# DeepLearnPhysics/dynamic-gcnn

Hardware: AMD Instinct MI355X
Metric: point-clouds/sec fwd+bwd at (B,N,k,C)=(24,2048,20,3), 1/2/4/8 MI355X (higher is better)
Workload: dtype f32

## Files before the change

dynamic-gcnn_amd/csrc/knn.hip:

```cpp
#include "knn_common.h"
#include <type_traits>
#include <stdlib.h>

namespace {

constexpr int ROWS = 64;
constexpr int WAVES = 4;
constexpr int TJ = 128;
constexpr int PERW = TJ / WAVES;

struct DenseClouds {
  int N;
  __host__ __device__ constexpr DenseClouds(int n) : N(n) {}
  static constexpr bool kPacked = false;
  __device__ int64_t base(int b) const { return (int64_t)b * N; }
  __device__ int size(int) const { return N; }
};
struct PackedClouds {
  const int* __restrict__ off;
  int nseg;
  static constexpr bool kPacked = true;
  __device__ int64_t base(int b) const { return off[b]; }
  __device__ int size(int b) const { return off[b + 1] - off[b]; }
  __device__ int cloud_of(int64_t row) const {
// ... 667 lines not shown
    }
  }

  __syncthreads();
  float* md = reinterpret_cast<float*>(smem_raw);
  int* mj = reinterpret_cast<int*>(smem_raw) + ROWS * KC;
#pragma unroll 1
  for (int src = 1; src < 4; ++src) {
    if (src > 1) __syncthreads();
    if (lid == src) {
#pragma unroll
      for (int t = 0; t < KC; ++t) {
        md[t * ROWS + rslot] = dl[t];
        mj[t * ROWS + rslot] = jl[t];
      }
    }
    __syncthreads();
    if (cs == 0) {
#pragma unroll 1
      for (int t = 0; t < KC; ++t) {
        const float d = (h == 0) ? md[t * ROWS + rslot] : INFINITY;
        const int j = (h == 0) ? mj[t * ROWS + rslot] : 0x7fffffff;
        const lmask_t need = key_less<true>(d, j, dl[KC - 1], jl[KC - 1]);
        if (need == 0) break;
        list_insert<KC, true>(dl, jl, d, j);
      }
    }
  }
  if (lid == 0 && row < N) {
    int32_t* out = idx + ((int64_t)b * N + row) * k;
#pragma unroll
    for (int t = 0; t < KC; ++t)
      if (t < k) out[t] = jl[t];
  }
}

__device__ __forceinline__ unsigned long long knn_key(float d, int j) {
  const unsigned u = __float_as_uint(d + 0.0f);
  const unsigned o = (u & 0x80000000u) ? ~u : (u | 0x80000000u);
  return ((unsigned long long)o << 32) | (unsigned)j;
}
__device__ __forceinline__ float knn_key_dist(unsigned long long key) {
  const unsigned o = (unsigned)(key >> 32);
  return __uint_as_float((o & 0x80000000u) ? (o & 0x7fffffffu) : ~o);
}
__device__ __forceinline__ unsigned long long readlane64(unsigned long long v, int l) {
  const unsigned lo = __builtin_amdgcn_readlane((int)(unsigned)v, l), hi = __builtin_amdgcn_readlane((int)(unsigned)(v >> 32), l);
  return ((unsigned long long)hi << 32) | lo;
}

constexpr int KA_MAXE = 8;
constexpr int KA_SLACK = 192;
constexpr int KA_SLACK_LX = 64;
constexpr float KA_C1 = 0.5f * (1.0f - 1.0f / 8192.0f);
constexpr int KA_LEVELS = 7;
__device__ __forceinline__ constexpr float ka_level(int m) {
  constexpr float L[KA_LEVELS] = {1.0f, 0.9f, 0.81f, 0.729f, 0.6561f, 0.59049f, 0.531441f};
  return L[m];
}

template <int M>
__device__ __forceinline__ unsigned xchg32(unsigned v) {
  if constexpr (M == 1) return (unsigned)__builtin_amdgcn_update_dpp((int)v, (int)v, 0xB1, 0xF, 0xF, false);
  else if constexpr (M == 2) return (unsigned)__builtin_amdgcn_update_dpp((int)v, (int)v, 0x4E, 0xF, 0xF, false);
  else if constexpr (M == 4) {
    const int t = __builtin_amdgcn_update_dpp((int)v, (int)v, 0x104, 0xF, 0x5, false);
    return (unsigned)__builtin_amdgcn_update_dpp(t, (int)v, 0x114, 0xF, 0xA, false);
  } else if constexpr (M == 8) {
    const int t = __builtin_amdgcn_update_dpp((int)v, (int)v, 0x108, 0xF, 0x3, false);
    return (unsigned)__builtin_amdgcn_update_dpp(t, (int)v, 0x118, 0xF, 0xC, false);
  } else if constexpr (M == 16) return (unsigned)__builtin_amdgcn_ds_swizzle((int)v, 0x401F);
  else return __shfl_xor(v, M, 64);
}
template <int M>
__device__ __forceinline__ unsigned long long xchg64(unsigned long long v) {
  const unsigned lo = xchg32<M>((unsigned)v), hi = xchg32<M>((unsigned)(v >> 32));
  return ((unsigned long long)hi << 32) | lo;
}
template <int J2>
__device__ __forceinline__ unsigned long long bitonic_step(unsigned long long key, int lane, bool up) {
  const unsigned long long pk = xchg64<J2>(key);
  const bool take_min = ((lane & J2) == 0) == up;
  return (take_min == (pk < key)) ? pk : key;
}
template <int J2>
__device__ __forceinline__ unsigned long long bitonic_steps_down(unsigned long long key, int lane, bool up) {
  key = bitonic_step<J2>(key, lane, up);
  if constexpr (J2 > 1) key = bitonic_steps_down<J2 / 2>(key, lane, up);
  return key;
}
__device__ __forceinline__ unsigned long long wave_merge64(unsigned long long key, int lane) {
  return bitonic_steps_down<32>(key, lane, true);
}
__device__ __forceinline__ unsigned long long wave_sort64(unsigned long long key, int lane) {
  key = bitonic_steps_down<1>(key, lane, (lane & 2) == 0);
  key = bitonic_steps_down<2>(key, lane, (lane & 4) == 0);
  key = bitonic_steps_down<4>(key, lane, (lane & 8) == 0);
  key = bitonic_steps_down<8>(key, lane, (lane & 16) == 0);
  key = bitonic_steps_down<16>(key, lane, (lane & 32) == 0);
  return wave_merge64(key, lane);
}
template <int E>
__device__ __forceinline__ unsigned long long wave_lowest64(const unsigned long long (&key)[E], int S, int lane) {
  unsigned long long res = wave_sort64(key[0], lane);
#pragma unroll
  for (int q = 1; q < E; ++q) {
// ... 241 lines not shown
      for (int s = 0; s < 4; ++s) {
        const bf16x8 a1 = *reinterpret_cast<const bf16x8*>(base + 2 * s * CS);
        acc = __builtin_amdgcn_mfma_f32_32x32x16_bf16(a1, q1[s], acc, 0, 0, 0);
        if (NPR == 3) {
          const bf16x8 a2 = *reinterpret_cast<const bf16x8*>(base + PB + 2 * s * CS);
          acc = __builtin_amdgcn_mfma_f32_32x32x16_bf16(a1, q2[s], acc, 0, 0, 0);
          acc = __builtin_amdgcn_mfma_f32_32x32x16_bf16(a2, q1[s], acc, 0, 0, 0);
        }
      }
      const float thr = (row < N) ? thr_s[rslot] : -INFINITY;
      const float gi = si * C1 - 0.5f * thr;
      const float* sj = sjs + cbase + 4 * h;
      unsigned mask = 0u;
#pragma unroll
      for (int q = 0; q < 4; ++q) {
        const float4 s4 = *reinterpret_cast<const float4*>(sj + 8 * q);
        const float sv[4] = {s4.x, s4.y, s4.z, s4.w};
#pragma unroll
        for (int e = 0; e < 4; ++e) {
          const int r = 4 * q + e;
          mask |= sel_01(m_flt(sv[e] + gi, acc[r])) << r;
        }
      }
      while (true) {
        const bool has = mask != 0u;
        const unsigned long long bal = __ballot(has);
        if (bal == 0ull) break;
        const int g = __builtin_ctz(mask | 0x80000000u) & 15;
        const int before = __builtin_amdgcn_mbcnt_hi((unsigned)(bal >> 32), __builtin_amdgcn_mbcnt_lo((unsigned)bal, 0u));
        if (has) {
          const unsigned ci = (unsigned)(cbase + (g & 3) + 8 * (g >> 2) + 4 * h);
          myq[qn + before] = LX ? (qent_t)(((unsigned)l31 << 6) | ci) : (qent_t)(((unsigned)l31 << 27) | ((unsigned)j0 + ci));
          mask &= mask - 1u;
        }
        qn += __popcll(bal);
        if (qn >= 64) {
          process(64, j0, par);
          qn -= 64;
          const qent_t mv = myq[64 + lane];
          if (lane < qn) myq[lane] = mv;
        }
      }
      if (LX && qn > 0) {
        process(qn, j0, par);
        qn = 0;
      }
    }
  }
  if (qn > 0) process(qn, 0, (nt - 1) & 1);
  __syncthreads();
  if (tid < ROWS && row0 + tid < N) cnt[grow0 + tid] = cnt_s[tid];
}

__global__ __launch_bounds__(256) void knn_select_kernel(const unsigned long long* __restrict__ ent, const int* __restrict__ cnt,
                                                         int64_t rows, int cap, int k, int32_t* __restrict__ idx) {
  const int lane = threadIdx.x & 63;
  const int64_t row = (int64_t)blockIdx.x * 4 + (threadIdx.x >> 6);
  if (row >= rows) return;
  const int S = cnt[row];
  const unsigned long long* buf = ent + row * cap;
  int32_t* out = idx + row * k;
  if (S <= 64) {
    unsigned long long key = (lane < S) ? buf[lane] : ~0ull;
    key = wave_sort64(key, lane);
    if (lane < k) out[lane] = (int32_t)(unsigned)key;
    return;
  }
  unsigned long long key[KA_MAXE];
#pragma unroll
  for (int q = 0; q < KA_MAXE; ++q) {
    const int e = lane + 64 * q;
    key[q] = (e < S) ? buf[e] : ~0ull;
  }
  const unsigned long long best = wave_lowest64<KA_MAXE>(key, S, lane);
  if (lane < k) out[lane] = (int32_t)(unsigned)best;
}

int g_knn_bf16f = -1;
int knn_bf16f_mode() {
  if (g_knn_bf16f < 0) {
    const char* e = getenv("DGCNN_KNN_BF16F");
    g_knn_bf16f = e ? ((e[0] == 'a') ? 2 : atoi(e)) : 2;
  }
  return g_knn_bf16f;
}

int g_knn_valu = 0;
bool knn_force_valu() { return g_knn_valu == 1; }

template <int LP, int MAXSTEPS, class Clouds = DenseClouds>
__global__ __launch_bounds__(256) void knn_seed_bound_kernel(const float* __restrict__ x, const float* __restrict__ sq, Clouds cl,
                                                             int64_t ldx, const int32_t* __restrict__ seed, int64_t ldseed, int k,
                                                             int64_t rows, float* __restrict__ tau0) {
  constexpr int PPS = 64 / LP;
  constexpr int RW = 2;
  const int lane = threadIdx.x & 63;
  const int64_t per = ((rows + 7) / 8 + 4 * RW - 1) / (4 * RW) * (4 * RW);
  const int64_t g0 = (int64_t)(blockIdx.x & 7) * per + ((int64_t)(blockIdx.x >> 3) * 4 + (threadIdx.x >> 6)) * RW;
  if (g0 >= rows || ((int64_t)(blockIdx.x >> 3) * 4 + (threadIdx.x >> 6)) * RW >= per) return;
  const int slot = lane / LP, cq = lane % LP;
  const int steps = (k + PPS - 1) / PPS;
  int jj[RW], nn[RW];
  int64_t gr[RW];
  const float* xc[RW];
  const float* sc[RW];
#pragma unroll
// ... 167 lines not shown
}

extern "C" int64_t dgcnn_knn_workspace_bytes(int B, int N, int C, int k) {
  if (B <= 0 || N <= 0) return 0;
  size_t n = 2 * knn_sq_bytes(B, N);
  if (dg::knn_grid_applicable(C, k)) n += dg::knn_grid_workspace_bytes(B, N);
  else if (knn_append_shape(C, k)) n += knn_append_bytes(B, N, k);
  return (int64_t)n;
}

static int g_knn_seed_min_n = -2;
static int knn_seed_min_n() {
  if (g_knn_seed_min_n == -2) {
    const char* e = getenv("DGCNN_KNN_SEED_MIN_N");
    g_knn_seed_min_n = e ? atoi(e) : -1;
  }
  return g_knn_seed_min_n;
}
extern "C" int dgcnn_knn_seed_min_n(int n) {
  const int prev = knn_seed_min_n();
  if (n >= -1) g_knn_seed_min_n = n;
  return prev;
}

static int g_knn_append = -1;
static bool knn_append_on() {
  if (g_knn_append < 0) {
    const char* e = getenv("DGCNN_KNN_APPEND");
    g_knn_append = e ? atoi(e) : 1;
  }
  return g_knn_append != 0;
}
extern "C" int dgcnn_knn_append(int on) {
  const int prev = knn_append_on() ? 1 : 0;
  if (on >= 0) g_knn_append = on ? 1 : 0;
  return prev;
}

static int g_knn_npr[2] = {-1, -1};
static int knn_append_products(bool lx) {
  if (g_knn_npr[0] < 0) {
    int a = 1, b = 1;
    const char* e = getenv("DGCNN_KNN_APPEND_NPR");
    if (e) sscanf(e, "%d,%d", &a, &b);
    g_knn_npr[0] = (a == 3) ? 3 : 1;
    g_knn_npr[1] = (b == 3) ? 3 : 1;
  }
  return g_knn_npr[lx ? 0 : 1];
}
extern "C" int dgcnn_knn_append_products(int n) {
  const int prev = knn_append_products(true);
  if (n == 1 || n == 3) g_knn_npr[0] = g_knn_npr[1] = n;
  return prev;
}

static int g_knn_hist = -1;
static int knn_hist_stride(int N) {
  if (g_knn_hist < 0) {
    const char* e = getenv("DGCNN_KNN_HIST");
    g_knn_hist = e ? atoi(e) : 2;
    if (g_knn_hist != 0 && g_knn_hist != 1 && g_knn_hist != 2 && g_knn_hist != 4) g_knn_hist = 2;
  }
  return N >= 256 ? g_knn_hist : 0;
}
extern "C" int dgcnn_knn_hist(int stride) {
  const int prev = knn_hist_stride(1 << 20);
  if (stride == 0 || stride == 1 || stride == 2 || stride == 4) g_knn_hist = stride;
  return prev;
}

static int knn_impl(const char* what, const float* x, int B, int N, int C, int64_t ldx, int k, const int32_t* seed, int64_t ldseed,
                    int kseed, int32_t* idx, void* ws, size_t ws_bytes, void* stream) {
  DG_REQUIRE(x && idx && ws, DGCNN_EINVAL, "%s: null pointer", what);
  DG_REQUIRE(B > 0 && N > 0 && C > 0 && ldx >= C, DGCNN_EINVAL, "%s: bad shape B=%d N=%d C=%d", what, B, N, C);
  DG_REQUIRE(k > 0 && k <= N, DGCNN_EINVAL, "%s: k=%d must be in [1, N=%d] (tf.nn.top_k raises otherwise)", what, k, N);
  DG_REQUIRE(k <= 64, DGCNN_EUNSUP, "%s: k=%d > 64 unsupported", what, k);
  DG_REQUIRE(C <= 128, DGCNN_EUNSUP, "%s: C=%d > 128 unsupported", what, C);
  DG_REQUIRE((reinterpret_cast<uintptr_t>(ws) & 15) == 0 && ws_bytes >= knn_sq_bytes(B, N), DGCNN_EINVAL,
             "%s: workspace must be 16-byte aligned and hold dgcnn_knn_workspace_bytes(B, N, C, k) bytes (got %zu)", what, ws_bytes);
  hipStream_t st = (hipStream_t)stream;
  float* sq_ws = reinterpret_cast<float*>(ws);
  const int64_t rows = (int64_t)B * N;
  const int vec_ok = (ldx % 4 == 0) && ((reinterpret_cast<uintptr_t>(x) & 15) == 0);
  const size_t grid_off = 2 * knn_sq_bytes(B, N);
  const bool append = knn_append_on() && knn_append_shape(C, k) && vec_ok && !knn_force_valu() && knn_bf16f_mode() != 0 &&
                      ws_bytes >= grid_off + knn_append_bytes(B, N, k);
  const int min_n = knn_seed_min_n() >= 0 ? knn_seed_min_n() : (append ? 0 : 4096);
  const bool seeded = seed && kseed >= k && kseed <= 64 && C > 4 && C <= 64 && C % 4 == 0 && vec_ok && !knn_force_valu() &&
                      N >= min_n && (int64_t)N * ldx < ((int64_t)1 << 31) && ws_bytes >= 2 * knn_sq_bytes(B, N);
  const bool grid_ws = dg::knn_grid_applicable(C, k) && !knn_force_valu() && ws_bytes >= grid_off + dg::knn_grid_workspace_bytes(B, N);
  dg::launch(sqnorm_kernel, dim3((unsigned)dg::cdiv(rows, SQ_ROWS)), dim3(256), sizeof(float) * SQ_ROWS * (C + 1), st, x,
                     ldx, rows, C, sq_ws);
  if (grid_ws && N >= dg::knn_grid_min_n())
    return dg::launch_knn_grid(x, sq_ws, B, N, C, ldx, k, idx, reinterpret_cast<char*>(ws) + grid_off, st);
  float* tau0 = nullptr;
  if (seeded) {
    tau0 = reinterpret_cast<float*>(reinterpret_cast<char*>(ws) + knn_sq_bytes(B, N));
    if (!launch_seed_bound(x, sq_ws, rows, DenseClouds(N), C, ldx, seed, ldseed, k, tau0, st)) tau0 = nullptr;
  }
  if (tau0 && append) {
    char* base = reinterpret_cast<char*>(ws) + grid_off;
    int* cnt = reinterpret_cast<int*>(base);
    unsigned long long* ent = reinterpret_cast<unsigned long long*>(base + (((size_t)rows * sizeof(int) + 255) & ~(size_t)255));
    const int cap = knn_append_cap(k, N);
    const dim3 grid((unsigned)dg::cdiv(N, ROWS), (unsigned)B);
    const int npr = knn_append_products(knn_append_lx(N));
    const int tmask = knn_append_tighten_mask(knn_append_lx(N));
#define DG_KA(LXV, NPRV) dg::launch((knn_bf16a_kernel<LXV, NPRV>), grid, dim3(256), 0, st, x, (const float*)sq_ws, N, C, ldx, k, (const float*)tau0, cap, ent, cnt, tmask)
    if (knn_append_lx(N)) { if (npr == 1) DG_KA(true, 1); else DG_KA(true, 3); }
    else { if (npr == 1) DG_KA(false, 1); else DG_KA(false, 3); }
#undef DG_KA
    dg::launch(knn_select_kernel, dim3((unsigned)dg::cdiv(rows, 4)), dim3(256), 0, st, (const unsigned long long*)ent, (const int*)cnt, rows,
               cap, k, idx);
    return dg::check_launch(what);
  }
  if (C <= 4) {
    const int hs = knn_hist_stride(N);
    if (hs > 0 && !knn_force_valu() && k <= 64 && N >= 4 * k * hs && ws_bytes >= 2 * knn_sq_bytes(B, N)) {
      float* tb = reinterpret_cast<float*>(reinterpret_cast<char*>(ws) + knn_sq_bytes(B, N));
      const dim3 hg((unsigned)dg::cdiv(N, 64), (unsigned)B);
      if (hs == 1) dg::launch(knn_hist_bound_kernel<1>, hg, dim3(256), 0, st, x, (const float*)sq_ws, N, C, ldx, k, tb);
      else if (hs == 2) dg::launch(knn_hist_bound_kernel<2>, hg, dim3(256), 0, st, x, (const float*)sq_ws, N, C, ldx, k, tb);
      else dg::launch(knn_hist_bound_kernel<4>, hg, dim3(256), 0, st, x, (const float*)sq_ws, N, C, ldx, k, tb);
      tau0 = tb;
    }
    return dispatch_k<4>(x, sq_ws, B, N, C, ldx, k, vec_ok, idx, tau0, st);
  }
  if (C <= 16) return dispatch_k<16>(x, sq_ws, B, N, C, ldx, k, vec_ok, idx, tau0, st);
  if (C <= 64) return dispatch_k<64>(x, sq_ws, B, N, C, ldx, k, vec_ok, idx, tau0, st);
  return dispatch_k<128>(x, sq_ws, B, N, C, ldx, k, vec_ok, idx, tau0, st);
}

extern "C" int dgcnn_knn_f32(const float* x, int B, int N, int C, int64_t ldx, int k, int32_t* idx,
                             void* ws, size_t ws_bytes, void* stream) {
  return knn_impl("dgcnn_knn_f32", x, B, N, C, ldx, k, nullptr, 0, 0, idx, ws, ws_bytes, stream);
}

extern "C" int dgcnn_knn_seeded_f32(const float* x, int B, int N, int C, int64_t ldx, int k, const int32_t* seed, int64_t ldseed,
                                    int kseed, int32_t* idx, void* ws, size_t ws_bytes, void* stream) {
  DG_REQUIRE(!seed || (ldseed >= kseed && kseed > 0), DGCNN_EINVAL, "dgcnn_knn_seeded_f32: bad seed shape");
  return knn_impl("dgcnn_knn_seeded_f32", x, B, N, C, ldx, k, seed, ldseed, kseed, idx, ws, ws_bytes, stream);
}

extern "C" int64_t dgcnn_knn_seg_workspace_bytes(int rows, int max_n, int C, int k) {
  if (rows <= 0 || max_n <= 0) return 0;
  size_t n = 2 * knn_sq_bytes(1, rows);
  if (knn_append_shape(C, k)) n += knn_append_rows_bytes((size_t)rows, knn_append_cap(k, max_n));
  return (int64_t)n;
}

extern "C" int dgcnn_knn_seg_f32(const float* x, int64_t ldx, int C, int k, int nseg, const int32_t* seg_off, int rows, int min_n,
                                 int max_n, const int32_t* seed, int64_t ldseed, int kseed, int32_t* idx, void* ws, size_t ws_bytes,
                                 void* stream) {
  const char* what = "dgcnn_knn_seg_f32";
  DG_REQUIRE(x && idx && ws && seg_off, DGCNN_EINVAL, "%s: null pointer", what);
  DG_REQUIRE(nseg > 0 && nseg <= 65535 && rows > 0 && C > 0 && ldx >= C, DGCNN_EINVAL, "%s: bad shape nseg=%d rows=%d C=%d", what,
             nseg, rows, C);
  DG_REQUIRE(min_n > 0 && min_n <= max_n && max_n <= rows && (int64_t)min_n * nseg <= rows && (int64_t)max_n * nseg >= rows,
             DGCNN_EINVAL, "%s: cloud sizes min_n=%d max_n=%d do not fit %d rows in %d clouds", what, min_n, max_n, rows, nseg);
  DG_REQUIRE(k > 0 && k <= min_n, DGCNN_EINVAL, "%s: k=%d must be in [1, smallest cloud=%d] (tf.nn.top_k raises otherwise)", what, k,
             min_n);
  DG_REQUIRE(k <= 64, DGCNN_EUNSUP, "%s: k=%d > 64 unsupported", what, k);
  DG_REQUIRE(C <= 128, DGCNN_EUNSUP, "%s: C=%d > 128 unsupported", what, C);
  DG_REQUIRE(!seed || (ldseed >= kseed && kseed > 0), DGCNN_EINVAL, "%s: bad seed shape", what);
  DG_REQUIRE((reinterpret_cast<uintptr_t>(ws) & 15) == 0 && ws_bytes >= knn_sq_bytes(1, rows), DGCNN_EINVAL,
             "%s: workspace must be 16-byte aligned and hold dgcnn_knn_seg_workspace_bytes(rows, max_n, C, k) bytes (got %zu)", what,
             ws_bytes);
  hipStream_t st = (hipStream_t)stream;
  float* sq_ws = reinterpret_cast<float*>(ws);
  float* tb = reinterpret_cast<float*>(reinterpret_cast<char*>(ws) + knn_sq_bytes(1, rows));
  const bool tb_ok = ws_bytes >= 2 * knn_sq_bytes(1, rows);
  const PackedClouds cl{seg_off, nseg};
  const int vec_ok = (ldx % 4 == 0) && ((reinterpret_cast<uintptr_t>(x) & 15) == 0);
  const size_t aux = 2 * knn_sq_bytes(1, rows);
  const bool lx = knn_append_lx(max_n);
  const int cap = knn_append_cap(k, max_n);
  const bool append = knn_append_on() && knn_append_shape(C, k) && vec_ok && !knn_force_valu() && knn_bf16f_mode() != 0 &&
                      ws_bytes >= aux + knn_append_rows_bytes((size_t)rows, cap);
  const int seed_min = knn_seed_min_n() >= 0 ? knn_seed_min_n() : 0;
  const bool seeded = append && seed && kseed >= k && kseed <= 64 && min_n >= seed_min && (int64_t)max_n * ldx < ((int64_t)1 << 31);
  dg::launch(sqnorm_kernel, dim3((unsigned)dg::cdiv(rows, SQ_ROWS)), dim3(256), sizeof(float) * SQ_ROWS * (C + 1), st, x, ldx,
             (int64_t)rows, C, sq_ws);
  if (seeded && launch_seed_bound(x, sq_ws, (int64_t)rows, cl, C, ldx, seed, ldseed, k, tb, st)) {
    char* base = reinterpret_cast<char*>(ws) + aux;
    int* cnt = reinterpret_cast<int*>(base);
    unsigned long long* ent = reinterpret_cast<unsigned long long*>(base + (((size_t)rows * sizeof(int) + 255) & ~(size_t)255));
    const dim3 grid((unsigned)dg::cdiv(max_n, ROWS), (unsigned)nseg);
    const int npr = knn_append_products(lx);
    const int tmask = knn_append_tighten_mask(lx);
#define DG_KA(LXV, NPRV) dg::launch((knn_bf16a_kernel<LXV, NPRV, PackedClouds>), grid, dim3(256), 0, st, x, (const float*)sq_ws, cl, C, ldx, k, (const float*)tb, cap, ent, cnt, tmask)
    if (lx) { if (npr == 1) DG_KA(true, 1); else DG_KA(true, 3); }
    else { if (npr == 1) DG_KA(false, 1); else DG_KA(false, 3); }
#undef DG_KA
    dg::launch(knn_select_kernel, dim3((unsigned)dg::cdiv(rows, 4)), dim3(256), 0, st, (const unsigned long long*)ent, (const int*)cnt,
               (int64_t)rows, cap, k, idx);
    return dg::check_launch(what);
  }
  if (C <= 4) {
    const int hs = knn_hist_stride(min_n);
    const float* tau0 = nullptr;
    if (hs > 0 && !knn_force_valu() && min_n >= 4 * k * hs && tb_ok) {
      const dim3 hg((unsigned)dg::cdiv(max_n, 64), (unsigned)nseg);
      if (hs == 1) dg::launch(knn_hist_bound_kernel<1, PackedClouds>, hg, dim3(256), 0, st, x, (const float*)sq_ws, cl, C, ldx, k, tb);
      else if (hs == 2) dg::launch(knn_hist_bound_kernel<2, PackedClouds>, hg, dim3(256), 0, st, x, (const float*)sq_ws, cl, C, ldx, k, tb);
      else dg::launch(knn_hist_bound_kernel<4, PackedClouds>, hg, dim3(256), 0, st, x, (const float*)sq_ws, cl, C, ldx, k, tb);
      tau0 = tb;
    }
    return dispatch_k_packed<4>(x, sq_ws, cl, max_n, C, ldx, k, vec_ok, idx, tau0, st);
  }
  if (C <= 16) return dispatch_k_packed<16>(x, sq_ws, cl, max_n, C, ldx, k, vec_ok, idx, nullptr, st);
  if (C <= 64) return dispatch_k_packed<64>(x, sq_ws, cl, max_n, C, ldx, k, vec_ok, idx, nullptr, st);
  return dispatch_k_packed<128>(x, sq_ws, cl, max_n, C, ldx, k, vec_ok, idx, nullptr, st);
}
```

dynamic-gcnn_amd/dgcnn/_hip.py:

```python
from __future__ import annotations

import ctypes
import os

import torch

_HERE = os.path.dirname(os.path.abspath(__file__))
LIB_PATH = os.environ.get("DGCNN_HIP_LIB") or os.path.join(_HERE, "libdgcnn_hip.so")
STAT_SLOTS = 32

c_int, c_i64, c_f32, c_f64, c_vp, c_sz, c_u64 = (ctypes.c_int, ctypes.c_int64, ctypes.c_float, ctypes.c_double,
                                                  ctypes.c_void_p, ctypes.c_size_t, ctypes.c_uint64)

PROTOTYPES = {
    "dgcnn_version": [],
    "dgcnn_last_error": [],
    "dgcnn_knn_workspace_bytes": [c_int, c_int, c_int, c_int],
    "dgcnn_knn_grid": [c_int],
    "dgcnn_knn_force_valu": [c_int],
    "dgcnn_knn_bf16_filter": [c_int],
    "dgcnn_knn_f32": [c_vp, c_int, c_int, c_int, c_i64, c_int, c_vp, c_vp, c_sz, c_vp],
    "dgcnn_knn_seed_min_n": [c_int],
    "dgcnn_knn_append": [c_int],
    "dgcnn_knn_append_products": [c_int],
    "dgcnn_knn_hist": [c_int],
    "dgcnn_knn_seeded_f32": [c_vp, c_int, c_int, c_int, c_i64, c_int, c_vp, c_i64, c_int, c_vp, c_vp, c_sz, c_vp],
    "dgcnn_knn_seg_workspace_bytes": [c_int, c_int, c_int, c_int],
    "dgcnn_knn_seg_f32": [c_vp, c_i64, c_int, c_int, c_int, c_vp, c_int, c_int, c_int, c_vp, c_i64, c_int, c_vp, c_vp, c_sz, c_vp],
    "dgcnn_edge_gather_f32": [c_vp, c_i64, c_vp, c_int, c_int, c_int, c_int, c_vp, c_vp],
    "dgcnn_edge_gather_bwd_f32": [c_vp, c_vp, c_int, c_int, c_int, c_int, c_vp, c_i64, c_vp],
    "dgcnn_edge_mlp_f32": [c_vp, c_i64, c_vp, c_vp, c_int, c_int, c_int, c_int, c_int, c_vp, c_vp, c_vp],
    "dgcnn_edge_mlp_wgrad_f32": [c_vp, c_i64, c_vp, c_vp, c_int, c_int, c_int, c_int, c_int, c_vp, c_f32,
                                 c_vp, c_sz, c_vp],
    "dgcnn_edge_mlp_dgrad_scatter_f32": [c_vp, c_vp, c_vp, c_int, c_int, c_int, c_int, c_int, c_vp, c_i64, c_vp],
    "dgcnn_edge_nbr_gemm_f32": [c_vp, c_i64, c_vp, c_vp, c_vp, c_i64, c_int, c_int, c_int, c_int, c_int, c_vp, c_vp, c_vp],
    "dgcnn_edge_nbr_wgrad_f32": [c_vp, c_i64, c_vp, c_vp, c_int, c_int, c_int, c_int, c_int, c_vp, c_f32,
                                 c_vp, c_sz, c_vp],
    "dgcnn_edge_csr_build": [c_vp, c_int, c_int, c_int, c_vp, c_vp, c_vp, c_vp],
    "dgcnn_edge_gather_sum_f32": [c_vp, c_vp, c_vp, c_i64, c_int, c_vp, c_i64, c_vp],
    "dgcnn_edge_weight_split_f32": [c_vp, c_int, c_int, c_vp, c_vp],
    "dgcnn_edge_gather_add_f32": [c_vp, c_i64, c_vp, c_i64, c_vp, c_int, c_int, c_int, c_int, c_vp, c_vp, c_vp],
    "dgcnn_edge_wgrad_combine_f32": [c_vp, c_int, c_int, c_vp, c_vp],
    "dgcnn_edge_bn_act_kreduce_f32": [c_vp, c_i64, c_vp, c_i64, c_vp, c_int, c_int, c_int, c_int, c_vp, c_vp, c_vp,
                                      c_int, c_vp, c_i64, c_vp, c_i64, c_vp, c_vp],
    "dgcnn_edge_bn_bwd_reduce_f32": [c_vp, c_i64, c_vp, c_i64, c_vp, c_int, c_int, c_int, c_int, c_vp, c_vp, c_vp,
                                     c_int, c_vp, c_i64, c_vp, c_i64, c_vp, c_i64, c_vp, c_vp, c_vp],
    "dgcnn_edge_bn_bwd_reduce_points_f32": [c_vp, c_i64, c_vp, c_i64, c_vp, c_vp, c_i64, c_vp, c_i64, c_vp, c_i64, c_int,
                                            c_int, c_vp, c_vp],
    "dgcnn_edge_bn_bwd_apply_f32": [c_vp, c_i64, c_vp, c_i64, c_vp, c_int, c_int, c_int, c_int, c_vp, c_vp, c_vp,
                                    c_int, c_vp, c_i64, c_vp, c_i64, c_vp, c_i64, c_vp, c_vp, c_vp, c_vp, c_i64, c_vp,
                                    c_f32, c_vp],
    "dgcnn_edge_bn_bwd_apply_wgrad_f32": [c_vp, c_i64, c_vp, c_i64, c_vp, c_int, c_int, c_int, c_int, c_vp, c_vp, c_vp,
                                          c_vp, c_i64, c_vp, c_i64, c_vp, c_i64, c_vp, c_vp, c_vp, c_i64, c_int, c_vp, c_vp, c_f32,
                                          c_vp, c_sz, c_vp],
    "dgcnn_bn1_act_dropout_f32": [c_vp, c_i64, c_int, c_vp, c_vp, c_vp, c_int, c_f32, c_vp, c_vp, c_i64, c_vp],
    "dgcnn_bn1_bwd_dropout_f32": [c_vp, c_i64, c_int, c_vp, c_vp, c_vp, c_int, c_f32, c_vp, c_vp, c_i64, c_vp, c_vp, c_vp, c_f32, c_vp],
    "dgcnn_set_stat_slots": [c_int],
    "dgcnn_get_stat_slots": [],
    "dgcnn_gemm_set_arith": [c_int],
    "dgcnn_gemm_get_arith": [],
    "dgcnn_gemm_stat_writers": [c_int, c_int, c_int, c_int, c_vp, c_i64, c_vp, c_i64],
    "dgcnn_gemm_x3_tile_rows": [c_int, c_int, c_int],
    "dgcnn_gemm_x3_tile_cols": [c_int, c_int, c_int],
    "dgcnn_gemm_x3_tile_override": [c_int],
    "dgcnn_gemm_f32": [c_int, c_int, c_int, c_int, c_int, c_vp, c_i64, c_vp, c_i64, c_vp, c_i64, c_f32,
                       c_vp, c_i64, c_int, c_vp, c_vp, c_int, c_vp, c_sz, c_vp],
    "dgcnn_colmax_decode_f32": [c_vp, c_i64, c_vp, c_vp, c_vp],
    "dgcnn_split_planes_f32": [c_vp, c_i64, c_i64, c_i64, c_int, c_int, c_vp, c_vp, c_i64, c_i64, c_vp],
    "dgcnn_planes_scale_f32": [c_vp, c_i64, c_i64, c_int, c_f32, c_vp, c_vp, c_vp],
    "dgcnn_gemm_planes_f32": [c_int, c_int, c_int, c_int, c_int, c_vp, c_i64, c_i64, c_vp, c_i64, c_i64, c_vp, c_vp, c_vp, c_i64, c_f32,
                              c_vp, c_i64, c_int, c_vp, c_vp, c_int, c_vp, c_sz, c_vp],
    "dgcnn_param_scales_f32": [c_vp, c_i64, c_f64, c_f32, c_vp, c_vp, c_vp],
    "dgcnn_bn_act_planes_f32": [c_vp, c_i64, c_i64, c_int, c_vp, c_vp, c_vp, c_int, c_int, c_vp, c_vp, c_i64, c_i64, c_vp, c_i64,
                                c_vp, c_i64, c_vp],
    "dgcnn_bn1_bwd_reduce_max_f32": [c_vp, c_i64, c_int, c_vp, c_vp, c_vp, c_int, c_vp, c_i64, c_vp, c_vp, c_vp],
    "dgcnn_bn1_bwd_apply_planes_f32": [c_vp, c_i64, c_int, c_vp, c_vp, c_vp, c_int, c_vp, c_i64, c_vp, c_vp, c_int, c_vp, c_vp,
                                       c_i64, c_i64, c_vp, c_vp, c_i64, c_int, c_vp, c_f32, c_vp],
# ... 250 lines not shown
```

include/dgcnn_hip.h:

```cpp
#ifndef DGCNN_HIP_H_
#define DGCNN_HIP_H_

#include <stddef.h>
#include <stdint.h>

#ifdef __cplusplus
extern "C" {
#endif

#define DGCNN_OK 0
#define DGCNN_EINVAL (-1)
#define DGCNN_ELAUNCH (-2)
#define DGCNN_ENOSPC (-3)
#define DGCNN_EUNSUP (-4)

#define DGCNN_STAT_SLOTS 32
int dgcnn_set_stat_slots(int n);
int dgcnn_get_stat_slots(void);

int dgcnn_version(void);
const char* dgcnn_last_error(void);

int64_t dgcnn_knn_workspace_bytes(int B, int N, int C, int k);
int dgcnn_knn_grid(int mode);
int dgcnn_knn_force_valu(int on);
int dgcnn_knn_bf16_filter(int mode);
int dgcnn_knn_f32(const float* x, int B, int N, int C, int64_t ldx, int k, int32_t* idx,
                  void* ws, size_t ws_bytes, void* stream);
int dgcnn_knn_seeded_f32(const float* x, int B, int N, int C, int64_t ldx, int k, const int32_t* seed, int64_t ldseed,
                         int kseed, int32_t* idx, void* ws, size_t ws_bytes, void* stream);
int dgcnn_knn_seed_min_n(int n);
int dgcnn_knn_append(int on);
int dgcnn_knn_append_products(int n);
int dgcnn_knn_hist(int stride);
int64_t dgcnn_knn_seg_workspace_bytes(int rows, int max_n, int C, int k);
int dgcnn_knn_seg_f32(const float* x, int64_t ldx, int C, int k, int nseg, const int32_t* seg_off, int rows, int min_n, int max_n,
                      const int32_t* seed, int64_t ldseed, int kseed, int32_t* idx, void* ws, size_t ws_bytes, void* stream);

int dgcnn_edge_mlp_bf16_supported(int C, int k, int F);
int dgcnn_edge_mlp_bf16_bwd_supported(int C, int k, int F);
int64_t dgcnn_edge_mlp_bf16_bwd_workspace_bytes(int B, int N, int C, int k, int F);
int dgcnn_edge_mlp_bf16_bwd(const float* x, int64_t ldx, const int32_t* idx, const float* W0, int B, int N, int C, int k, int F,
                            const float* mean, const float* rstd, const float* beta, const float* mx, int64_t ldmx,
                            const float* cnt, const float* dmx, int64_t lddmx, const float* dmn, int64_t lddmn, double* red,
                            void* dYb, float* dysum, int64_t lddysum, float* dW0, float* dbeta, float dbeta_beta, void* ws,
                            size_t ws_bytes, void* stream);
int dgcnn_edge_gather_sum_bf16(const void* dY, const int32_t* off, const int32_t* rev, int64_t R, int F, float* S, int64_t lds,
                               void* stream);
int dgcnn_round_bf16_f32(const float* src, float* dst, int64_t n, void* stream);
int dgcnn_edge_mlp_bf16(const float* x, int64_t ldx, const int32_t* idx, const float* W0, int B, int N, int C, int k, int F,
                        float* Y, void* stream);
int dgcnn_edge_mlp_bf16_stats(const float* x, int64_t ldx, const int32_t* idx, const float* W0, int B, int N, int C, int k, int F,
                              double* stats, void* stream);
int dgcnn_edge_mlp_bf16_bn_kreduce(const float* x, int64_t ldx, const int32_t* idx, const float* W0, int B, int N, int C, int k,
                                   int F, const float* mean, const float* rstd, const float* beta, float* mx, int64_t ldmx,
                                   float* mn, int64_t ldmn, float* cnt, int pack_cnt, void* stream);

int dgcnn_edge_gather_f32(const float* x, int64_t ldx, const int32_t* idx, int B, int N, int C, int k,
                          float* E, void* stream);
int dgcnn_edge_gather_bwd_f32(const float* dE, const int32_t* idx, int B, int N, int C, int k,
                              float* dx, int64_t lddx, void* stream);

int dgcnn_edge_mlp_f32(const float* x, int64_t ldx, const int32_t* idx, const float* W0,
                       int B, int N, int C, int k, int F, float* Y, double* stats, void* stream);
int dgcnn_edge_mlp_wgrad_f32(const float* x, int64_t ldx, const int32_t* idx, const float* dY,
                             int B, int N, int C, int k, int F, float* dW0, float beta,
                             void* ws, size_t ws_bytes, void* stream);
int dgcnn_edge_mlp_dgrad_scatter_f32(const float* dY, const float* W0, const int32_t* idx,
                                     int B, int N, int C, int k, int F, float* dx, int64_t lddx,
                                     void* stream);

int dgcnn_edge_nbr_gemm_f32(const float* x, int64_t ldx, const int32_t* idx, const float* Wb,
                            const float* U, int64_t ldu, int B, int N, int C, int k, int F,
                            float* Y, double* stats, void* stream);
int dgcnn_edge_nbr_wgrad_f32(const float* x, int64_t ldx, const int32_t* idx, const float* dY,
                             int B, int N, int C, int k, int F, float* dWb, float beta,
                             void* ws, size_t ws_bytes, void* stream);

int dgcnn_edge_csr_build(const int32_t* idx, int B, int N, int k, int32_t* cnt_ws, int32_t* off,
                         int32_t* rev, void* stream);
int dgcnn_edge_gather_sum_f32(const float* dY, const int32_t* off, const int32_t* rev, int64_t R, int F,
                              float* S, int64_t lds, void* stream);

int dgcnn_edge_weight_split_f32(const float* W0, int C, int F, float* Wcat, void* stream);
int dgcnn_edge_gather_add_f32(const float* V, int64_t ldv, const float* U, int64_t ldu, const int32_t* idx,
                              int B, int N, int k, int F, float* Y, double* stats, void* stream);
// ... 162 lines not shown
```

Measured before the change: 5521.

## Add wide-tile bf16 MFMA append kNN kernel for large-channel layers

Adds a new append-mode kNN kernel that stages 128-candidate tiles of up to 64 channels in swizzled shared memory. Each wave computes a 32x64 distance block with bf16 MFMA. The kernel register-prefetches the next tile, re-scores filtered candidates in exact fp32 from shared memory, and remaps blocks across the grid in an interleaved order. It is enabled by default for the LX (large channel) path in both the dense and packed entry points. The aim is better reuse of candidate loads and higher MFMA throughput in the dynamic-graph kNN for deeper layers, at the cost of more shared memory and an added occupancy hint.

```diff
diff --git a/dynamic-gcnn_amd/csrc/knn.hip b/dynamic-gcnn_amd/csrc/knn.hip
--- a/dynamic-gcnn_amd/csrc/knn.hip
+++ b/dynamic-gcnn_amd/csrc/knn.hip
@@ -743,6 +743,7 @@
 constexpr int KA_MAXE = 8;
 constexpr int KA_SLACK = 192;
 constexpr int KA_SLACK_LX = 64;
+constexpr int KW_TJ = 128;
 constexpr float KA_C1 = 0.5f * (1.0f - 1.0f / 8192.0f);
 constexpr int KA_LEVELS = 7;
 __device__ __forceinline__ constexpr float ka_level(int m) {
@@ -1090,6 +1091,307 @@
   if (tid < ROWS && row0 + tid < N) cnt[grow0 + tid] = cnt_s[tid];
 }
 
+template <int NPR, class Clouds = DenseClouds>
+__global__ __launch_bounds__(256, 3) void knn_bf16w_kernel(const float* __restrict__ x, const float* __restrict__ sq, Clouds cl, int C,
+                                                           int64_t ldx, int k, const float* __restrict__ tau0, int cap,
+                                                           unsigned long long* __restrict__ ent, int* __restrict__ cnt,
+                                                           int ka_tight_mask, int nclouds) {
+  using f32x16 = __attribute__((ext_vector_type(16))) float;
+  constexpr int CP = 64;
+  constexpr int TW = KW_TJ;
+  constexpr int QN = 128;
+  constexpr unsigned SH_B = 4 * (TW * CP + ROWS * CP + 2 * TW + ROWS + ROWS + 4 * ROWS) + 2 * 4 * QN + 16;
+  __shared__ __attribute__((aligned(16))) char smem_raw[SH_B];
+  float* xc = reinterpret_cast<float*>(smem_raw);
+  float* xq = xc + TW * CP;
+  float* sjs = xq + ROWS * CP;
+  float* sjr = sjs + TW;
+  volatile float* thr_s = sjr + TW;
+  int* cnt_s = reinterpret_cast<int*>(const_cast<float*>(thr_s) + ROWS);
+  unsigned* hist = reinterpret_cast<unsigned*>(cnt_s + ROWS);
+  volatile unsigned short* queue = reinterpret_cast<unsigned short*>(hist + 4 * ROWS);
+  volatile int* flags = reinterpret_cast<int*>(const_cast<unsigned short*>(queue) + 4 * QN);
+
+  int bx, b;
+  if constexpr (Clouds::kPacked) {
+    bx = blockIdx.x;
+    b = blockIdx.y;
+  } else {
+    const int nbx = (cl.size(0) + ROWS - 1) / ROWS;
+    const int total = nbx * nclouds;
+    const int per = (total + 7) / 8;
+    const int lg = (int)(blockIdx.x & 7) * per + (int)(blockIdx.x >> 3);
+    if (lg >= total) return;
+    b = lg / nbx;
+    bx = lg - b * nbx;
+  }
+  const int tid = threadIdx.x;
+  const int lane = tid & 63;
+  const int w = tid >> 6;
+  const int l31 = lane & 31, h = lane >> 5;
+  const int qg = w & 1;
+  const int cs = w >> 1;
+  const int N = cl.size(b);
+  if (Clouds::kPacked && bx * ROWS >= N) return;
+  const int row0 = bx * ROWS;
+  const int row = row0 + qg * 32 + l31;
+  const float* xb = x + cl.base(b) * ldx;
+  const float* sqb = sq + cl.base(b);
+  const int rowc = row < N ? row : N - 1;
+  const int rslot = qg * 32 + l31;
+  const float si = sqb[rowc];
+  const float* xi_row = xb + (int64_t)rowc * ldx;
+  const int64_t grow0 = cl.base(b) + row0;
+  const int trig = cap - KW_TJ;
+  volatile unsigned short* myq = queue + w * QN;
+  constexpr float C1 = (NPR == 3) ? KA_C1 : 0.5f * (1.0f - 1.0f / 64.0f);
+  const int tight_mask = ka_tight_mask;
+
+  bf16x8 q1[4], q2[4];
+#pragma unroll
+  for (int s = 0; s < 4; ++s) {
+    float v[8];
+#pragma unroll
+    for (int e = 0; e < 2; ++e) {
+      const int c = 16 * s + 8 * h + 4 * e;
+      float4 t4 = make_float4(0.f, 0.f, 0.f, 0.f);
+      if (c < C) t4 = *reinterpret_cast<const float4*>(xi_row + c);
+      v[4 * e] = t4.x; v[4 * e + 1] = t4.y; v[4 * e + 2] = t4.z; v[4 * e + 3] = t4.w;
+    }
+    unsigned hh[4], mm[4];
+#pragma unroll
+    for (int e = 0; e < 4; ++e) {
+      if constexpr (NPR == 3) split2_pair(v[2 * e], v[2 * e + 1], hh[e], mm[e]);
+      else { hh[e] = cvt_pk_bf16(v[2 * e], v[2 * e + 1]); mm[e] = 0u; }
+    }
+    const uint4 H4 = make_uint4(hh[0], hh[1], hh[2], hh[3]), M4 = make_uint4(mm[0], mm[1], mm[2], mm[3]);
+    q1[s] = *reinterpret_cast<const bf16x8*>(&H4);
+    q2[s] = *reinterpret_cast<const bf16x8*>(&M4);
+  }
+  for (int e = tid; e < ROWS * (CP / 4); e += 256) {
+    const int r = e / (CP / 4), c4 = (e % (CP / 4)) * 4;
+    const int rr = (row0 + r < N) ? row0 + r : N - 1;
+    float4 t4 = make_float4(0.f, 0.f, 0.f, 0.f);
+    if (c4 < C) t4 = *reinterpret_cast<const float4*>(xb + (int64_t)rr * ldx + c4);
+    *reinterpret_cast<float4*>(xq + r * CP + ((((c4 >> 2) ^ r) & 15) << 2)) = t4;
+  }
+  if (tid < ROWS) {
+    const int rr = (row0 + tid < N) ? row0 + tid : N - 1;
+    const float t0 = tau0[cl.base(b) + rr];
+    thr_s[tid] = next_up(t0);
+    cnt_s[tid] = 0;
+    const bool lv = (t0 > 1e-30f) && (t0 < INFINITY) && (N <= 65536);
+    hist[4 * tid] = lv ? (__float_as_uint(t0) >> 16) : 0u;
+    hist[4 * tid + 1] = 0u; hist[4 * tid + 2] = 0u; hist[4 * tid + 3] = 0u;
+  }
+  if (tid < 2) flags[tid] = 0;
+
+  const int fr = tid >> 4, fc4 = (tid & 15) << 2;
+  const int fsw = ((tid & 15) ^ fr) << 2;
+  constexpr int NV = (TW * (CP / 4)) / 256;
+  float4 pre[NV];
+  float pre_s = INFINITY;
+  auto fetch = [&](int j0) {
+#pragma unroll
+    for (int i = 0; i < NV; ++i) {
+      const int j = j0 + fr + 16 * i;
+      const int jc = j < N ? j : N - 1;
+      const int cc = fc4 < C ? fc4 : C - 4;
+      const float4 t4 = *reinterpret_cast<const float4*>(xb + (int64_t)jc * ldx + cc);
+      const bool ok = fc4 < C;
+      pre[i] = make_float4(ok ? t4.x : 0.f, ok ? t4.y : 0.f, ok ? t4.z : 0.f, ok ? t4.w : 0.f);
+    }
+    if (tid < TW) pre_s = (j0 + tid < N) ? sqb[j0 + tid] : INFINITY;
+  };
+  auto stash = [&]() {
+#pragma unroll
+    for (int i = 0; i < NV; ++i) *reinterpret_cast<float4*>(xc + (fr + 16 * i) * CP + fsw) = pre[i];
+    if (tid < TW) {
+      sjs[tid] = pre_s * C1;
+      sjr[tid] = pre_s;
+    }
+  };
+
+  auto process = [&](int nvalid, int j0, int par) {
+    const bool on = lane < nvalid;
+    const unsigned e = on ? (unsigned)myq[lane] : 0u;
+    const int rl = (int)(e >> 7);
+    const int jl = (int)(e & 127u);
+    const int j = j0 + jl;
+    const int rs = qg * 32 + rl;
+    const float* xi = xq + rs * CP;
+    const int rx = (rs & 15) << 2;
+    const float* xj = xc + jl * CP;
+    const int jx = (jl & 15) << 2;
+    const float sjv = sjr[jl];
+    float p = 0.f;
+    if (C == 64) {
+      float4 v[3], a[3];
+      v[0] = *reinterpret_cast<const float4*>(xj + (0 ^ jx));
+      v[1] = *reinterpret_cast<const float4*>(xj + (4 ^ jx));
+      a[0] = *reinterpret_cast<const float4*>(xi + (0 ^ rx));
+      a[1] = *reinterpret_cast<const float4*>(xi + (4 ^ rx));
+#pragma unroll
+      for (int q = 0; q < 16; ++q) {
+        if (q + 2 < 16) {
+          a[(q + 2) % 3] = *reinterpret_cast<const float4*>(xi + ((4 * (q + 2)) ^ rx));
+          v[(q + 2) % 3] = *reinterpret_cast<const float4*>(xj + ((4 * (q + 2)) ^ jx));
+        }
+        const float4 aa = a[q % 3], vv = v[q % 3];
+        p = fmaf(aa.x, vv.x, p); p = fmaf(aa.y, vv.y, p); p = fmaf(aa.z, vv.z, p); p = fmaf(aa.w, vv.w, p);
+      }
+    } else {
+#pragma unroll 2
+      for (int c0 = 0; c0 < C; c0 += 4) {
+        const float4 aa = *reinterpret_cast<const float4*>(xi + (c0 ^ rx));
+        const float4 vv = *reinterpret_cast<const float4*>(xj + (c0 ^ jx));
+        p = fmaf(aa.x, vv.x, p); p = fmaf(aa.y, vv.y, p); p = fmaf(aa.z, vv.z, p); p = fmaf(aa.w, vv.w, p);
+      }
+    }
+    const float sir = __shfl(si, rl, 64);
+    const float tt = sir + sjv;
+    const float tp = 2.0f * p;
+    const float d = tt - tp;
+    if (on && d < thr_s[rs]) {
+      const int pos = atomicAdd(&cnt_s[rs], 1);
+      ent[(grow0 + rs) * cap + pos] = knn_key(d, Clouds::kPacked ? (int)cl.base(b) + j : j);
+      if (pos >= trig) flags[par] = 1;
+      const float T = __uint_as_float(hist[4 * rs] << 16);
+      int m = 0;
+#pragma unroll
+      for (int u = 0; u < KA_LEVELS; ++u) m += (d < T * ka_level(u)) ? 1 : 0;
+      if (m > 0 && j != row0 + rs) atomicAdd(&hist[4 * rs + (m >> 1)], 1u << ((m & 1) << 4));
+    }
+  };
+
+  const int nt = (N + TW - 1) / TW;
+  fetch(0);
+  const int rsw = l31 & 15;
+  int qn = 0;
+
+#pragma unroll 1
+  for (int t = 0; t < nt; ++t) {
+    const int j0 = t * TW;
+    const int par = t & 1;
+    __syncthreads();
+    stash();
+    if (t + 1 < nt) fetch(j0 + TW);
+    if (tid == 0) flags[par] = 0;
+    if (t > 0 && ((t & tight_mask) == 0 || t < 4) && lane < 16) {
+      const int r = w + 4 * lane;
+      const uint4 hw = *reinterpret_cast<const uint4*>(hist + 4 * r);
+      const float T = __uint_as_float(hw.x << 16);
+      const unsigned bin[KA_LEVELS] = {hw.x >> 16, hw.y & 0xffffu, hw.y >> 16, hw.z & 0xffffu, hw.z >> 16, hw.w & 0xffffu, hw.w >> 16};
+      unsigned c = 0u;
+      float tn = INFINITY;
+#pragma unroll
+      for (int u = KA_LEVELS - 1; u >= 0; --u) {
+        c += bin[u];
+        if (c >= (unsigned)k && tn == INFINITY) tn = T * ka_level(u);
+      }
+      if (T > 0.f && tn < thr_s[r]) thr_s[r] = tn;
+    }
+    if (t > 0 && flags[par ^ 1]) {
+#pragma unroll 1
+      for (int r = w; r < ROWS; r += 4) {
+        const int S = cnt_s[r];
+        if (S > trig) {
+          unsigned long long* buf = ent + (grow0 + r) * cap;
+          unsigned long long key[KA_MAXE];
+#pragma unroll
+          for (int q = 0; q < KA_MAXE; ++q) {
+            const int e = lane + 64 * q;
+            key[q] = (e < S) ? __hip_atomic_load(buf + e, __ATOMIC_RELAXED, __HIP_MEMORY_SCOPE_AGENT) : ~0ull;
+          }
+          const unsigned long long best = wave_lowest64<KA_MAXE>(key, S, lane);
+          if (lane < k) buf[lane] = best;
+          if (lane == k - 1) {
+            thr_s[r] = next_up(knn_key_dist(best));
+            cnt_s[r] = k;
+          }
+        }
+      }
+    }
+    __syncthreads();
+    if (j0 + cs * 64 < N) {
+      f32x16 acc0, acc1;
+#pragma unroll
+      for (int r = 0; r < 16; ++r) { acc0[r] = 0.f; acc1[r] = 0.f; }
+      const float* xr0 = xc + (cs * 64 + l31) * CP;
+      const float* xr1 = xr0 + 32 * CP;
+#pragma unroll
+      for (int s = 0; s < 4; ++s) {
+        const int g0 = ((4 * s + 2 * h) ^ rsw) << 2, g1 = ((4 * s + 2 * h + 1) ^ rsw) << 2;
+        const float4 u0 = *reinterpret_cast<const float4*>(xr0 + g0), u1 = *reinterpret_cast<const float4*>(xr0 + g1);
+        const float4 w0 = *reinterpret_cast<const float4*>(xr1 + g0), w1 = *reinterpret_cast<const float4*>(xr1 + g1);
+        unsigned ha[4], ma[4], hb[4], mb[4];
+        if constexpr (NPR == 3) {
+          split2_pair(u0.x, u0.y, ha[0], ma[0]); split2_pair(u0.z, u0.w, ha[1], ma[1]);
+          split2_pair(u1.x, u1.y, ha[2], ma[2]); split2_pair(u1.z, u1.w, ha[3], ma[3]);
+          split2_pair(w0.x, w0.y, hb[0], mb[0]); split2_pair(w0.z, w0.w, hb[1], mb[1]);
+          split2_pair(w1.x, w1.y, hb[2], mb[2]); split2_pair(w1.z, w1.w, hb[3], mb[3]);
+        } else {
+          ha[0] = cvt_pk_bf16(u0.x, u0.y); ha[1] = cvt_pk_bf16(u0.z, u0.w); ha[2] = cvt_pk_bf16(u1.x, u1.y); ha[3] = cvt_pk_bf16(u1.z, u1.w);
+          hb[0] = cvt_pk_bf16(w0.x, w0.y); hb[1] = cvt_pk_bf16(w0.z, w0.w); hb[2] = cvt_pk_bf16(w1.x, w1.y); hb[3] = cvt_pk_bf16(w1.z, w1.w);
+        }
+        const uint4 HA = make_uint4(ha[0], ha[1], ha[2], ha[3]), HB = make_uint4(hb[0], hb[1], hb[2], hb[3]);
+        const bf16x8 a1 = *reinterpret_cast<const bf16x8*>(&HA), b1 = *reinterpret_cast<const bf16x8*>(&HB);
+        acc0 = __builtin_amdgcn_mfma_f32_32x32x16_bf16(a1, q1[s], acc0, 0, 0, 0);
+        acc1 = __builtin_amdgcn_mfma_f32_32x32x16_bf16(b1, q1[s], acc1, 0, 0, 0);
+        if constexpr (NPR == 3) {
+          const uint4 MA = make_uint4(ma[0], ma[1], ma[2], ma[3]), MB = make_uint4(mb[0], mb[1], mb[2], mb[3]);
+          const bf16x8 a2 = *reinterpret_cast<const bf16x8*>(&MA), b2 = *reinterpret_cast<const bf16x8*>(&MB);
+          acc0 = __builtin_amdgcn_mfma_f32_32x32x16_bf16(a1, q2[s], acc0, 0, 0, 0);
+          acc1 = __builtin_amdgcn_mfma_f32_32x32x16_bf16(b1, q2[s], acc1, 0, 0, 0);
+          acc0 = __builtin_amdgcn_mfma_f32_32x32x16_bf16(a2, q1[s], acc0, 0, 0, 0);
+          acc1 = __builtin_amdgcn_mfma_f32_32x32x16_bf16(b2, q1[s], acc1, 0, 0, 0);
+        }
+      }
+      const float thr = (row < N) ? thr_s[rslot] : -INFINITY;
+      const float gi = si * C1 - 0.5f * thr;
+      const float* sj = sjs + cs * 64 + 4 * h;
+      unsigned mask = 0u;
+#pragma unroll
+      for (int q = 0; q < 4; ++q) {
+        const float4 s4 = *reinterpret_cast<const float4*>(sj + 8 * q);
+        const float4 z4 = *reinterpret_cast<const float4*>(sj + 32 + 8 * q);
+        const float sv[4] = {s4.x, s4.y, s4.z, s4.w}, zv[4] = {z4.x, z4.y, z4.z, z4.w};
+#pragma unroll
+        for (int e = 0; e < 4; ++e) {
+          const int r = 4 * q + e;
+          mask |= sel_01(m_flt(sv[e] + gi, acc0[r])) << r;
+          mask |= sel_01(m_flt(zv[e] + gi, acc1[r])) << (16 + r);
+        }
+      }
+      while (true) {
+        const bool has = mask != 0u;
+        const unsigned long long bal = __ballot(has);
+        if (bal == 0ull) break;
+        const int before = __builtin_amdgcn_mbcnt_hi((unsigned)(bal >> 32), __builtin_amdgcn_mbcnt_lo((unsigned)bal, 0u));
+        if (has) {
+          const int g = __builtin_ctz(mask);
+          const unsigned ci = (unsigned)(cs * 64 + 32 * (g >> 4) + (g & 3) + 8 * ((g >> 2) & 3) + 4 * h);
+          myq[qn + before] = (unsigned short)(((unsigned)l31 << 7) | ci);
+          mask &= mask - 1u;
+        }
+        qn += __popcll(bal);
+        if (qn >= 64) {
+          process(64, j0, par);
+          qn -= 64;
+          const unsigned short mv = myq[64 + lane];
+          if (lane < qn) myq[lane] = mv;
+        }
+      }
+      if (qn > 0) {
+        process(qn, j0, par);
+        qn = 0;
+      }
+    }
+  }
+  __syncthreads();
+  if (tid < ROWS && row0 + tid < N) cnt[grow0 + tid] = cnt_s[tid];
+}
+
 __global__ __launch_bounds__(256) void knn_select_kernel(const unsigned long long* __restrict__ ent, const int* __restrict__ cnt,
                                                          int64_t rows, int cap, int k, int32_t* __restrict__ idx) {
   const int lane = threadIdx.x & 63;
@@ -1363,6 +1665,24 @@
   const int prev = knn_append_products(true);
   if (n == 1 || n == 3) g_knn_npr[0] = g_knn_npr[1] = n;
   return prev;
+}
+
+static int g_knn_wide = -1;
+static bool knn_append_wide() {
+  if (g_knn_wide < 0) {
+    const char* e = getenv("DGCNN_KNN_WIDE");
+    g_knn_wide = e ? (atoi(e) != 0) : 1;
+  }
+  return g_knn_wide != 0;
+}
+extern "C" int dgcnn_knn_append_wide(int on) {
+  const int prev = knn_append_wide() ? 1 : 0;
+  if (on >= 0) g_knn_wide = on ? 1 : 0;
+  return prev;
+}
+static int knn_wide_tighten_mask() {
+  const int every = (knn_append_tighten_mask(true) + 1) / 2;
+  return (every > 1 ? every : 1) - 1;
 }
 
 static int g_knn_hist = -1;
@@ -1418,9 +1738,15 @@
     const int npr = knn_append_products(knn_append_lx(N));
     const int tmask = knn_append_tighten_mask(knn_append_lx(N));
 #define DG_KA(LXV, NPRV) dg::launch((knn_bf16a_kernel<LXV, NPRV>), grid, dim3(256), 0, st, x, (const float*)sq_ws, N, C, ldx, k, (const float*)tau0, cap, ent, cnt, tmask)
-    if (knn_append_lx(N)) { if (npr == 1) DG_KA(true, 1); else DG_KA(true, 3); }
+#define DG_KW(NPRV) dg::launch((knn_bf16w_kernel<NPRV>), wgrid, dim3(256), 0, st, x, (const float*)sq_ws, DenseClouds(N), C, ldx, k, (const float*)tau0, cap, ent, cnt, wmask, B)
+    if (knn_append_lx(N) && knn_append_wide()) {
+      const dim3 wgrid((unsigned)(8 * dg::cdiv(dg::cdiv(N, ROWS) * B, 8)));
+      const int wmask = knn_wide_tighten_mask();
+      if (npr == 1) DG_KW(1); else DG_KW(3);
+    } else if (knn_append_lx(N)) { if (npr == 1) DG_KA(true, 1); else DG_KA(true, 3); }
     else { if (npr == 1) DG_KA(false, 1); else DG_KA(false, 3); }
 #undef DG_KA
+#undef DG_KW
     dg::launch(knn_select_kernel, dim3((unsigned)dg::cdiv(rows, 4)), dim3(256), 0, st, (const unsigned long long*)ent, (const int*)cnt, rows,
                cap, k, idx);
     return dg::check_launch(what);
@@ -1500,9 +1826,12 @@
     const int npr = knn_append_products(lx);
     const int tmask = knn_append_tighten_mask(lx);
 #define DG_KA(LXV, NPRV) dg::launch((knn_bf16a_kernel<LXV, NPRV, PackedClouds>), grid, dim3(256), 0, st, x, (const float*)sq_ws, cl, C, ldx, k, (const float*)tb, cap, ent, cnt, tmask)
-    if (lx) { if (npr == 1) DG_KA(true, 1); else DG_KA(true, 3); }
+#define DG_KW(NPRV) dg::launch((knn_bf16w_kernel<NPRV, PackedClouds>), grid, dim3(256), 0, st, x, (const float*)sq_ws, cl, C, ldx, k, (const float*)tb, cap, ent, cnt, knn_wide_tighten_mask(), nseg)
+    if (lx && knn_append_wide()) { if (npr == 1) DG_KW(1); else DG_KW(3); }
+    else if (lx) { if (npr == 1) DG_KA(true, 1); else DG_KA(true, 3); }
     else { if (npr == 1) DG_KA(false, 1); else DG_KA(false, 3); }
 #undef DG_KA
+#undef DG_KW
     dg::launch(knn_select_kernel, dim3((unsigned)dg::cdiv(rows, 4)), dim3(256), 0, st, (const unsigned long long*)ent, (const int*)cnt,
                (int64_t)rows, cap, k, idx);
     return dg::check_launch(what);
diff --git a/dynamic-gcnn_amd/dgcnn/_hip.py b/dynamic-gcnn_amd/dgcnn/_hip.py
--- a/dynamic-gcnn_amd/dgcnn/_hip.py
+++ b/dynamic-gcnn_amd/dgcnn/_hip.py
@@ -23,6 +23,7 @@
     "dgcnn_knn_seed_min_n": [c_int],
     "dgcnn_knn_append": [c_int],
     "dgcnn_knn_append_products": [c_int],
+    "dgcnn_knn_append_wide": [c_int],
     "dgcnn_knn_hist": [c_int],
     "dgcnn_knn_seeded_f32": [c_vp, c_int, c_int, c_int, c_i64, c_int, c_vp, c_i64, c_int, c_vp, c_vp, c_sz, c_vp],
     "dgcnn_knn_seg_workspace_bytes": [c_int, c_int, c_int, c_int],
diff --git a/include/dgcnn_hip.h b/include/dgcnn_hip.h
--- a/include/dgcnn_hip.h
+++ b/include/dgcnn_hip.h
@@ -32,6 +32,7 @@
 int dgcnn_knn_seed_min_n(int n);
 int dgcnn_knn_append(int on);
 int dgcnn_knn_append_products(int n);
+int dgcnn_knn_append_wide(int on);
 int dgcnn_knn_hist(int stride);
 int64_t dgcnn_knn_seg_workspace_bytes(int rows, int max_n, int C, int k);
 int dgcnn_knn_seg_f32(const float* x, int64_t ldx, int C, int k, int nseg, const int32_t* seg_off, int rows, int min_n, int max_n,
```

Result: no change. 5574 (median of 6 runs) (+1.0%).
